# iangitonga/tinyllama.cpp

Hardware: AMD Instinct MI355X
Metric: decode tok/s TinyLlama-1.1B q4 ctx=2048, 1 GPU; achieved HBM GB/s vs peak (higher is better)
Workload: dtype q4 weights x q8 activations (int8 dot, f32 accumulate); 1 GPU; TinyLlama-1.1B q4 greedy single-token decode, batch 1 per GPU, steps end at n=2048 (BASELINE.json configs[3]); ctx=2048, graph=True, steps_per_graph_replay=4, kv_cache=q8 blocks (reference layout), argmax=device, parallelism=replicas x1

## Files before the change

### tinyllama.cpp_amd/csrc/gten_decode.hip

```cpp
#include "gten_dev.h"
#include "gten_rt.h"
#include "gten_hip_sample.h"

#include <cmath>
#include <vector>
#include <algorithm>

using namespace gtd;

extern __shared__ __attribute__((aligned(16))) uint8_t g_smem[];

#define DEC_CHUNK 256
#define DEC_MAX_LANES 4
#define DEC_ATT_MAXCH 8
#define GEMVM_F16_LDS_LIMIT 65536

static int g_only_family = -1;
#define DEC_LAUNCH(tag, kernel, grid, block, smem, ...)                                        \
    do {                                                                                       \
        if (g_only_family < 0 || g_only_family == (tag)) GTR_LAUNCH(tag, kernel, grid, block, smem, __VA_ARGS__); \
    } while (0)

#define DEC_LAUNCH_HOT(tag, kernel, grid, block, smem, hw, a) \
    DEC_LAUNCH(tag, kernel, grid, block, smem, (hw).w[0], (hw).w[1], (hw).w[2], (hw).w[3], (hw).w[4], (hw).w[5], (hw).w[6], a)

struct DecStep {
    int n;
    int advance;
    int stop;
};


struct ActStage {
    float* row;
    float* red;
    ActQ8 q8;
};

__device__ __forceinline__ ActStage carve_stage(int d)
{
    ActStage s;
    s.red = (float*)g_smem;
    s.row = (float*)(g_smem + 64);
    s.q8 = actq8_carve(g_smem + 64 + (size_t)d * 4, d >> 5);
    return s;
}
static size_t stage_bytes(int d) { return 64 + (size_t)d * 4 + (size_t)(d >> 5) * 40; }

enum { PRO_EMBED = 0, PRO_RESID = 1, PRO_ATT = 2, PRO_ATTW = 3, PRO_ACTQ8 = 4 };
enum { EPI_RAW = 0, EPI_SILUMUL = 1, EPI_STAGE = 2, EPI_STAGE_FRAG = 3 };

#define WXP_PLANES 8
#include "gten_decode_wx.h"
#include "gten_decode_wide_wx.h"
#include "gten_decode_ffn.h"
#include "gten_decode_wxp.h"
#include "gten_decode_attn.h"
#include "gten_decode_attn_exact64.h"
#include "gten_decode_attn_wide.h"
#include "gten_decode_attn_hm.h"
#include "gten_decode_sample.h"


using namespace gtr;

struct gten_hip_decoder {
    gten_hip_decoder_desc d;
    std::vector<gten_hip_layer_ptrs> layers;
    DecStep* step = nullptr;
    int32_t* tokens = nullptr;
    int32_t* result = nullptr;
    int32_t* ids_stage = nullptr;
    float *qkv_raw = nullptr, *proj_raw = nullptr, *down_raw = nullptr;
    float *scores = nullptr, *stats = nullptr, *att_part = nullptr;
    uint8_t *xbuf = nullptr, *hbuf = nullptr;
    float* act_f = nullptr;
    int8_t* act_q = nullptr;
    float* act_d = nullptr;
    int* act_sum = nullptr;
    float* best_val = nullptr;
    int* best_idx = nullptr;
    int n_best = 0;
    std::vector<DecStep> slots;
    int dev_n = -1;
    std::vector<int> dev_ns;
    int only_family = -1;
    int n_seq = 1;
    const void** kv_tab = nullptr;
    std::vector<const void*> kv_real;
    std::vector<char> kv_parked;
    void* dummy_kv = nullptr;
    int8_t* stg_q = nullptr;
    float* stg_d = nullptr;
    int* stg_sum = nullptr;
    float* stg_f = nullptr;
    float* logits_m = nullptr;
    float* gu_raw = nullptr;
    int n_chunks = 0;
    hipGraph_t graph = nullptr;
    hipGraphExec_t exec = nullptr;
    hipGraph_t graph_k = nullptr;
    hipGraphExec_t exec_k = nullptr;
    hipGraph_t graph_m[1 << DEC_MAX_LANES] = {}, graph_km[1 << DEC_MAX_LANES] = {};
    hipGraphExec_t exec_m[1 << DEC_MAX_LANES] = {}, exec_km[1 << DEC_MAX_LANES] = {};
    SampleParam* samp = nullptr;
    std::vector<SampleParam> samp_host;
    int n_sampling = 0;
    hipGraph_t s_graph = nullptr, s_graph_k = nullptr, s_graph_m[1 << DEC_MAX_LANES] = {}, s_graph_km[1 << DEC_MAX_LANES] = {};
    hipGraphExec_t s_exec = nullptr, s_exec_k = nullptr, s_exec_m[1 << DEC_MAX_LANES] = {}, s_exec_km[1 << DEC_MAX_LANES] = {};
    unsigned lane_mask = 0;
    int last_run_lanes = 0;
    const float2* rope = nullptr;
    float2* rope_now = nullptr;
    bool exact = false;
    bool persist_on = false;
    struct PersistState* persist = nullptr;
    uint8_t* hm = nullptr;
    size_t hm_seq_stride = 0, hm_cache_bytes = 0, hm_chunk_bytes = 0;
    std::vector<char> hm_dirty;
    unsigned long long hm_imports = 0, hm_import_launches = 0;
    unsigned long long watch_epoch = 0;
    bool watch_foreign = false;
    int lanes = 1;
    hipStream_t lane_stream[DEC_MAX_LANES] = {nullptr, nullptr, nullptr, nullptr};
    hipEvent_t lane_fork = nullptr, lane_join[DEC_MAX_LANES] = {nullptr, nullptr, nullptr, nullptr};
};

struct LaneBufs {
    int n_seq;
    DecStep* step; int32_t* tokens; int32_t* result; const SampleParam* samp;
    float *qkv_raw, *proj_raw, *down_raw, *scores, *stats, *att_part;
    uint8_t *xbuf, *hbuf;
    float* act_f; int8_t* act_q; float* act_d; int* act_sum;
    const void** kv_tab;
    int8_t* stg_q; float* stg_d; int* stg_sum; float* stg_f;
    float* logits_m; float* gu_raw; float2* rope_now;
};
static LaneBufs lane_bufs(const gten_hip_decoder* dc, int lane)
{
    const gten_hip_decoder_desc& d = dc->d;
    const size_t SL = (size_t)(dc->n_seq / dc->lanes), o = (size_t)lane * SL;
    const size_t E = (size_t)d.n_embd, F = (size_t)d.n_ffn, dh = E / d.n_heads, KV = dh * d.n_kv_heads, V = (size_t)d.n_vocab;
    const size_t planes = dc->n_seq >= 16 ? 2 : 1, H = (size_t)d.n_heads, C = (size_t)dc->n_chunks;
    LaneBufs b;
    b.n_seq = (int)SL;
    b.step = dc->step + o; b.tokens = dc->tokens + o * (d.max_ctx + 1); b.result = dc->result + o * (d.max_ctx + 2); b.samp = dc->samp + o;
    const size_t rplanes = dc->n_seq >= 16 ? (size_t)WXP_PLANES : 1;
    b.qkv_raw = dc->qkv_raw + o * rplanes * (E + 2 * KV);
    b.proj_raw = dc->proj_raw + o * rplanes * E; b.down_raw = dc->down_raw + o * rplanes * E;
    b.scores = dc->scores + o * H * d.max_ctx; b.stats = dc->stats + o * H * C * 2; b.att_part = dc->att_part + o * H * C * dh;
    b.xbuf = dc->xbuf + o * E * 4; b.hbuf = dc->hbuf + o * E * 4;
    b.act_f = dc->act_f + o * F; b.act_q = dc->act_q + o * 2 * F; b.act_d = dc->act_d + o * (F / 32); b.act_sum = dc->act_sum + o * (F / 32);
    b.kv_tab = dc->kv_tab ? dc->kv_tab + o * d.n_layers * 2 : nullptr;
    b.stg_q = dc->stg_q ? dc->stg_q + o * 2 * E : nullptr; b.stg_d = dc->stg_d ? dc->stg_d + o * (E / 32) : nullptr;
    b.stg_sum = dc->stg_sum ? dc->stg_sum + o * (E / 32) : nullptr; b.stg_f = dc->stg_f ? dc->stg_f + o * E : nullptr;
    b.logits_m = dc->logits_m ? dc->logits_m + o * V : nullptr; b.gu_raw = dc->gu_raw ? dc->gu_raw + o * planes * 2 * F : nullptr;
    b.rope_now = dc->rope_now + o * (dh / 2);
    return b;
}

static bool g_decode_exact = false;
static bool g_exact_now = false;
static bool g_lane_skip = false;
static bool g_kv_head_major = true;
extern "C" int gten_hip_set_kv_head_major(int on)
{
    g_kv_head_major = on != 0;
    return 0;
}
extern "C" int gten_hip_set_decode_exact(int on)
{
    g_decode_exact = on != 0;
    return 0;
}

static bool attention_grouped_ok(const AttnArgs& t, int n_seq)
{
    const int grp = t.n_heads / t.n_kv;
    const int min_seq = 8;
    if (t.adtype == GTEN_F16 && n_seq < 16) return false;
    return n_seq >= min_seq && (t.adtype == GTEN_Q8 || t.adtype == GTEN_F16) && t.d_head == 64 && (grp == 8 || grp == 4 || grp == 2 || grp == 1);
}

static int grp_shift1_of(int n_heads, int n_kv)
{
    const int grp = n_heads / n_kv;
    return (grp > 0 && (grp & (grp - 1)) == 0) ? __builtin_ctz(grp) + 1 : 0;
}

static bool attention_one_pass(int d_head);

static bool grouped_mm(const AttnArgs& t, int n_seq)
{
    return n_seq >= 16 && t.adtype == GTEN_Q8 && t.d_head == 64 && !g_exact_now;
}

static bool grouped_hm_f16(const AttnArgs& t, int n_seq)
{
    return n_seq >= 16 && t.adtype == GTEN_F16 && t.d_head == 64 && t.hm_k && !g_exact_now;
}

static bool grouped_one_pass(const AttnArgs& t, int n_seq)
{
    if (grouped_mm(t, n_seq) || grouped_hm_f16(t, n_seq)) return true;
    return attention_one_pass(t.d_head) && t.adtype == GTEN_Q8 && n_seq <= 8;
}

template <int GRP, int ADT>
static int launch_attention_g(const AttnArgs& t, int n_seq)
{
    constexpr size_t NW = (ADT == GTEN_Q8) ? 17 : 32;
    const dim3 grid(n_seq, t.n_chunks, t.n_kv);
    if constexpr (ADT == GTEN_Q8) if (grouped_mm(t, n_seq) && t.hm_k) {
        const int n_cq = (t.n_chunks + HM_WAVES - 1) / HM_WAVES;
        if (n_seq >= 128) DEC_LAUNCH(KT_DEC_ATTN_SCORE, (k_dec_attn_hm<GRP, true>), dim3(n_seq * n_cq * t.n_kv), dim3(64 * HM_WAVES), 2048, t, n_seq, n_cq);
        else DEC_LAUNCH(KT_DEC_ATTN_SCORE, (k_dec_attn_hm<GRP, false>), dim3(n_seq * n_cq * t.n_kv), dim3(64 * HM_WAVES), 2048, t, n_seq, n_cq);
        return 0;
    }
    if constexpr (ADT == GTEN_Q8) if (grouped_mm(t, n_seq)) {
        const size_t smem = (size_t)DEC_CHUNK * 68 + 2 * 8 * 264 * 2 + 16 * 64 + 32 * 4 + 8 * 4 + (size_t)4 * (DEC_MAXGRP + 2) * 2 + 128 + 128 * 4 + 80 + 64;
        GTR_REQUIRE((n_seq * t.n_chunks) % 8 == 0, "decoder: %d sequences x %d chunks is not a multiple of 8", n_seq, t.n_chunks);
        DEC_LAUNCH(KT_DEC_ATTN_SCORE, (k_dec_attn_mm_g<GRP>), dim3(n_seq * t.n_chunks * t.n_kv), dim3(256), smem, t, n_seq);
        return 0;
    }
    if constexpr (ADT == GTEN_Q8) if (grouped_one_pass(t, n_seq)) {
        constexpr size_t GP = (GRP + 1) / 2;
        const size_t smem = (size_t)(8 * GRP + 4 * GRP + 8 + 64) * 4 + (size_t)4 * (GRP + 2) * 2 + (size_t)(GRP + 2) * 64 + 16 +
// ... 19 lines not shown
        const size_t smem_m = (size_t)(128 + 16) * 4 + 128 + 128 + 64 + 16 + (size_t)17 * 64 * 2 + 64;
        DEC_LAUNCH(KT_DEC_ATTN_SCORE, (k_dec_attn_score_gm_f16<GRP>), grid, dim3(256), smem_m, t);
    } else if (ADT == GTEN_F16) {
        AttnArgs t1 = t;
        t1.grp_shift1 = grp_shift1_of(t.n_heads, t.n_kv);
        const AttnHotWords none{{0, 0, 0, 0, 0, 0, 0}};
        const size_t smem_s = (size_t)(16 + 3 * 64 + 16) * 4 + 32 + (size_t)3 * 64 + 64;
        DEC_LAUNCH_HOT(KT_DEC_ATTN_SCORE, (k_dec_attn_score64<GTEN_F16, true>), dim3(t.n_chunks, t.n_heads, n_seq), dim3(256), smem_s, none, t1);
    } else {
        DEC_LAUNCH(KT_DEC_ATTN_SCORE, (k_dec_attn_score_g<GRP, ADT>), grid, dim3(256), smem1, t);
    }
    if (exact) DEC_LAUNCH(KT_DEC_ATTN_PV, (k_dec_attn_pv_g<GRP, true, ADT>), grid, dim3(256), smem2, t);
    else DEC_LAUNCH(KT_DEC_ATTN_PV, (k_dec_attn_pv_g<GRP, false, ADT>), grid, dim3(256), smem2, t);
    return 0;
}

static int launch_attention_grouped(const AttnArgs& t, int n_seq)
{
    if (t.adtype == GTEN_Q8) {
        switch (t.n_heads / t.n_kv) {
        case 8: return launch_attention_g<8, GTEN_Q8>(t, n_seq);
        case 4: return launch_attention_g<4, GTEN_Q8>(t, n_seq);
        case 2: return launch_attention_g<2, GTEN_Q8>(t, n_seq);
        default: return launch_attention_g<1, GTEN_Q8>(t, n_seq);
        }
    }
    switch (t.n_heads / t.n_kv) {
    case 8: return launch_attention_g<8, GTEN_F16>(t, n_seq);
    case 4: return launch_attention_g<4, GTEN_F16>(t, n_seq);
    case 2: return launch_attention_g<2, GTEN_F16>(t, n_seq);
    default: return launch_attention_g<1, GTEN_F16>(t, n_seq);
    }
}

static bool attention_one_pass(int d_head)
{
    return d_head == 64 && !g_exact_now;
}

static int launch_attention(const AttnArgs& t0, dim3 agrid, size_t smem1)
{
    AttnArgs t = t0;
    t.grp_shift1 = grp_shift1_of(t.n_heads, t.n_kv);
    if (attention_one_pass(t.d_head)) {
        const size_t nw = (t.adtype == GTEN_Q8) ? 17 : 32;
        const size_t smem = 1152 + (size_t)2 * DEC_CHUNK * 4 + (size_t)DEC_CHUNK * nw * 4;
        const unsigned long long geo = (unsigned long long)(unsigned)t.kv_pitch | ((unsigned long long)(unsigned)t.max_ctx << 32);
        const unsigned long long heads = ((unsigned long long)(unsigned)t.n_heads << 32) | ((unsigned long long)(unsigned)t.n_kv << 40) |
                                         ((unsigned long long)(unsigned)t.grp_shift1 << 48);
        const AttnHotWords hw{{(unsigned long long)(uintptr_t)t.qkv_raw, (unsigned long long)(uintptr_t)t.rope_now, (unsigned long long)(uintptr_t)t.kcache,
                               (unsigned long long)(uintptr_t)t.step, geo, (unsigned long long)(unsigned)t.n_embd | heads, (unsigned long long)(uintptr_t)t.vcache}};
        const bool multi = agrid.z > 1 || t.kv_tab != nullptr;
        const dim3 g64(agrid.y, agrid.x, agrid.z);
        if (t.adtype == GTEN_Q8) {
            if (multi) DEC_LAUNCH_HOT(KT_DEC_ATTN_SCORE, (k_dec_attn_one64<GTEN_Q8, true>), g64, dim3(256), smem, hw, t);
            else DEC_LAUNCH_HOT(KT_DEC_ATTN_SCORE, (k_dec_attn_one64<GTEN_Q8, false>), g64, dim3(256), smem, hw, t);
        } else {
            if (multi) DEC_LAUNCH_HOT(KT_DEC_ATTN_SCORE, (k_dec_attn_one64<GTEN_F16, true>), g64, dim3(256), smem, hw, t);
            else DEC_LAUNCH_HOT(KT_DEC_ATTN_SCORE, (k_dec_attn_one64<GTEN_F16, false>), g64, dim3(256), smem, hw, t);
        }
        return 0;
    }
    if (t.d_head == 64) {
        const size_t nw = (t.adtype == GTEN_Q8) ? 17 : 32;
        const size_t smem2 = (size_t)2 * DEC_CHUNK * 4 + (size_t)DEC_CHUNK * nw * 4;
        const unsigned long long geo = (unsigned long long)(unsigned)t.kv_pitch | ((unsigned long long)(unsigned)t.max_ctx << 32);
        const unsigned long long heads = ((unsigned long long)(unsigned)t.n_heads << 32) | ((unsigned long long)(unsigned)t.n_kv << 40) |
                                         ((unsigned long long)(unsigned)t.grp_shift1 << 48);
        const AttnHotWords hs{{(unsigned long long)(uintptr_t)t.qkv_raw, (unsigned long long)(uintptr_t)t.rope_now, (unsigned long long)(uintptr_t)t.kcache,
                               (unsigned long long)(uintptr_t)t.step, geo, (unsigned long long)(unsigned)t.n_embd | heads, (unsigned long long)(uintptr_t)t.scores}};
        const AttnHotWords hp{{(unsigned long long)(uintptr_t)t.scores, (unsigned long long)(uintptr_t)t.stats, (unsigned long long)(uintptr_t)t.vcache,
                               (unsigned long long)(uintptr_t)t.step, geo, (unsigned long long)(unsigned)t.n_chunks | heads, (unsigned long long)(uintptr_t)t.att_part}};
        const bool multi = agrid.z > 1 || t.kv_tab != nullptr;
        const dim3 g64(agrid.y, agrid.x, agrid.z);
#define ATT_LAUNCH2(ADT, MULTI)                                                                                                          \
        do {                                                                                                                             \
            DEC_LAUNCH_HOT(KT_DEC_ATTN_SCORE, (k_dec_attn_score64<ADT, MULTI>), g64, dim3(256), smem1, hs, t);                           \
            DEC_LAUNCH_HOT(KT_DEC_ATTN_PV, (k_dec_attn_pv64<ADT, MULTI>), g64, dim3(256), smem2, hp, t);                                 \
        } while (0)
        if (t.adtype == GTEN_Q8) { if (multi) ATT_LAUNCH2(GTEN_Q8, true); else ATT_LAUNCH2(GTEN_Q8, false); }
        else { if (multi) ATT_LAUNCH2(GTEN_F16, true); else ATT_LAUNCH2(GTEN_F16, false); }
#undef ATT_LAUNCH2
        return 0;
    }
    DEC_LAUNCH(KT_DEC_ATTN_SCORE, k_dec_attn_score, agrid, dim3(256), smem1, t);
    DEC_LAUNCH(KT_DEC_ATTN_PV, k_dec_attn_pv, agrid, dim3(256), (size_t)2 * DEC_CHUNK * 4, t);
    return 0;
}

template <int WT, int PRO>
static GemvHotWords hot_of(const Gemv8Args& a)
{
    GemvHotWords hw;
    GemvHot& h = hw.h;
    if (PRO == PRO_RESID) { h.p0 = a.res_raw; h.p1 = a.res_a; h.p2 = a.norm_w; }
    else if (PRO == PRO_EMBED) { h.p0 = a.table; h.p1 = a.tokens; h.p2 = a.norm_w; }
    else if (PRO == PRO_ATT || PRO == PRO_ATTW) {
        h.p0 = a.att_part; h.p1 = (const void*)(uintptr_t)((unsigned)a.d_head_shift | ((unsigned)a.n_chunks << 8));
        h.p2 = (PRO == PRO_ATTW) ? a.att_stats : nullptr;
    }
    else { h.p0 = (WT == GTEN_F16) ? (const void*)a.act_f : (const void*)a.act_q; h.p1 = a.act_d; h.p2 = a.act_sum; }
    h.qs0 = a.qs[0]; h.ds0 = a.ds[0]; h.d_in = a.d_in; h.rows0 = a.rows[0]; h.step = a.step;
    return hw;
}

template <int WT, int PRO>
// ... 664 lines not shown
        }
        if (down_planes) {
            if ((rc = launch_wxp_f16(KT_DEC_GEMV_DOWN, (const uint16_t*)b.act_q, L.wdown, b.down_raw, F, E, S, E))) return rc;
        } else if ((rc = mmk(KT_DEC_GEMV_DOWN, b.act_q, b.act_d, b.down_raw, E, F, ks_of(F), L.wdown, E))) return rc;
    }
    Gemv8Args sf = base;
    sf.d_in = E; sf.res_a = hbuf; sf.res_raw = b.down_raw; sf.raw_stride = E; sf.norm_w = (const uint16_t*)d.final_norm;
    sf.raw_plane = (down_planes || ks_of(F) > 1) ? S * E : 0;
    sf.raw_nplanes = down_planes ? WXP_PLANES : 0;
    sf.act_q = b.stg_q; sf.act_d = b.stg_d; sf.act_sum = b.stg_sum; sf.act_f = b.stg_f;
    if ((rc = launch_stage_frag<WT, PRO_RESID>(KT_DEC_STAGE, sf, S))) return rc;
    if ((rc = mm(KT_DEC_GEMV_HEAD, b.stg_q, b.stg_d, b.stg_sum, b.logits_m, V, E, d.lm_head, V))) return rc;
    if (dc->n_sampling > 0)
        DEC_LAUNCH(KT_DEC_SAMPLE, k_dec_sample, dim3(S), dim3(SMP_THREADS), 0, (const float*)b.logits_m, V, V, b.samp,
                   b.step, b.result, d.max_ctx + 2, b.tokens, d.max_ctx + 1);
    else
        DEC_LAUNCH(KT_DEC_ARGMAX, k_dec_argmax, dim3(S), dim3(1024), 0, (const float*)b.logits_m, (const int*)nullptr,
                   V, b.step, b.result, V, d.max_ctx + 2, b.tokens, d.max_ctx + 1);
    return 0;
}

template <int WT>
static int enqueue_multi(gten_hip_decoder* dc, int lane)
{
    switch (dc->n_seq) {
    case 2: return enqueue_step_multi<WT, 2>(dc);
    case 4: return enqueue_step_multi<WT, 4>(dc);
    case 8: return enqueue_step_multi<WT, 8>(dc);
    }
    if (dc->n_seq >= 16) return enqueue_step_wide<WT>(dc, lane);
    return fail(-4, "decoder: n_seq %d not supported for this configuration", dc->n_seq);
}

#ifndef GTEN_WITH_PERSIST
#define GTEN_WITH_PERSIST 0
#endif
#if GTEN_WITH_PERSIST
#include "gten_decode_persist.h"
#else
struct PersistState {};
static bool g_persist_on = false;
extern "C" int gten_hip_set_decode_persistent(int on)
{
    if (on) return fail(-4, "set_decode_persistent: this library was built without the persistent step (-DGTEN_WITH_PERSIST=1, HISTORY.md)");
    return 0;
}
#endif

static int persist_prepare(gten_hip_decoder* dc);

static int enqueue_lane(gten_hip_decoder* dc, int lane)
{
    g_exact_now = dc->exact;
#if GTEN_WITH_PERSIST
    if (dc->persist_on && dc->n_seq == 1 && !dc->exact && (g_only_family < 0 || g_only_family == KT_DEC_PERSIST)) {
        if (int rc = persist_prepare(dc)) return rc;
        if (dc->persist) return persist_launch<GTEN_Q4>(dc->persist);
    }
#endif
    if (dc->n_seq > 1) {
        switch (dc->d.wdtype) {
        case GTEN_F16: return enqueue_multi<GTEN_F16>(dc, lane);
        case GTEN_Q8: return enqueue_multi<GTEN_Q8>(dc, lane);
        case GTEN_Q4: return enqueue_multi<GTEN_Q4>(dc, lane);
        }
    }
    switch (dc->d.wdtype) {
    case GTEN_F16: return enqueue_step_q8act<GTEN_F16>(dc);
    case GTEN_Q8: return enqueue_step_q8act<GTEN_Q8>(dc);
    case GTEN_Q4: return enqueue_step_q8act<GTEN_Q4>(dc);
    }
    return fail(-4, "decoder: bad weight dtype %d", dc->d.wdtype);
}

static int enqueue(gten_hip_decoder* dc, int count = 1)
{
    if (dc->lanes <= 1) {
        for (int i = 0; i < count; i++)
            if (int rc = enqueue_lane(dc, 0)) return rc;
        return 0;
    }
    const unsigned all = (1u << dc->lanes) - 1u, mask = (dc->lane_mask & all) ? (dc->lane_mask & all) : all;
    int g0 = 0;
    while (!((mask >> g0) & 1u)) g0++;
    const bool side = (mask & ~(1u << g0)) != 0;
    hipStream_t main_s = stream();
    if (side) {
        GTR_CHECK(hipEventRecord(dc->lane_fork, main_s));
        for (int g = g0 + 1; g < dc->lanes; g++)
            if ((mask >> g) & 1u) GTR_CHECK(hipStreamWaitEvent(dc->lane_stream[g], dc->lane_fork, 0));
    }
    int rc = 0;
    for (int g = g0; g < dc->lanes && !rc; g++) {
        if (!((mask >> g) & 1u)) continue;
        if (g != g0) gtr::stream_override(dc->lane_stream[g]);
        for (int i = 0; i < count && !rc; i++) rc = enqueue_lane(dc, g);
        gtr::stream_override(nullptr);
    }
    for (int g = g0 + 1; g < dc->lanes; g++) {
        if (!((mask >> g) & 1u)) continue;
        GTR_CHECK(hipEventRecord(dc->lane_join[g], dc->lane_stream[g]));
        GTR_CHECK(hipStreamWaitEvent(main_s, dc->lane_join[g], 0));
    }
    return rc;
}

static int decoder_build(gten_hip_decoder* dc, const gten_hip_decoder_desc& d, const gten_hip_layer_ptrs* layers,
                         const gten_hip_kv_ptrs* kv, int n_seq);

static int decoder_create_common(const gten_hip_decoder_desc* desc, const gten_hip_layer_ptrs* layers,
                                 const gten_hip_kv_ptrs* kv, int n_seq, gten_hip_decoder** out)
{
    GTR_NEED_INIT();
    GTR_REQUIRE(desc && layers && out, "decoder_create: null argument");
    const gten_hip_decoder_desc& d = *desc;
    GTR_REQUIRE(d.n_layers > 0 && d.n_heads > 0 && d.n_kv_heads > 0 && d.n_heads % d.n_kv_heads == 0, "decoder_create: bad head/layer counts");
    GTR_REQUIRE(d.n_embd % d.n_heads == 0, "decoder_create: n_embd %% n_heads != 0");
    const int dh = d.n_embd / d.n_heads;
    GTR_REQUIRE(dh == 32 || dh == 64, "decoder_create: fast path supports d_head 32 or 64 (got %d)", dh);
    GTR_REQUIRE(d.n_embd % 32 == 0 && d.n_ffn % 32 == 0 && d.n_embd <= 2048 && d.n_ffn <= 6144, "decoder_create: unsupported widths (n_embd <= 2048, n_ffn <= 6144)");
    GTR_REQUIRE(d.n_vocab > 0 && d.n_vocab <= 65535, "decoder_create: n_vocab %d outside [1, 65535] (row counts travel as 16-bit fields of the preloaded arguments)", d.n_vocab);
    GTR_REQUIRE(d.max_ctx > 0 && d.max_ctx <= GTEN_ROPE_MAX_POS, "decoder_create: max_ctx %d beyond the RoPE table", d.max_ctx);
    const bool pair_ok = (d.wdtype == GTEN_F16 && d.adtype == GTEN_F16) || ((d.wdtype == GTEN_Q8 || d.wdtype == GTEN_Q4) && d.adtype == GTEN_Q8);
    GTR_REQUIRE(pair_ok, "decoder_create: unsupported dtype pair (%d,%d) (tinyllama.cpp:258-265)", d.wdtype, d.adtype);
    GTR_REQUIRE(d.embed && d.final_norm && d.lm_head, "decoder_create: null model pointer");
    const bool wide = n_seq >= 16;
    GTR_REQUIRE(n_seq == 1 || n_seq == 2 || n_seq == 4 || n_seq == 8 || (wide && n_seq <= 64 && n_seq % 16 == 0) ||
                (n_seq > 64 && n_seq <= 64 * DEC_MAX_LANES && n_seq % 64 == 0) || (n_seq > 256 && n_seq <= 128 * DEC_MAX_LANES && n_seq % 128 == 0),
                "decoder_create: n_seq %d not in {1, 2, 4, 8, 16, 32, 48, 64, 128, 192, 256, 384, 512}", n_seq);
    GTR_REQUIRE(!wide || (d.n_ffn % 256 == 0 && d.n_embd % 256 == 0 && (dh * d.n_kv_heads) % 16 == 0),
                "decoder_create: n_seq >= 16 runs the W.x on the matrix cores: n_embd and n_ffn %% 256 == 0");
    GTR_REQUIRE(!wide || d.wdtype != GTEN_Q8 || d.n_ffn <= MMV_MAXP * 512,
                "decoder_create: q8 weights with n_seq >= 16 want n_ffn <= %d (the down projection's weight slab), got %d", MMV_MAXP * 512, d.n_ffn);
    GTR_REQUIRE(n_seq == 1 || (kv && dh == 64), "decoder_create: multi-sequence decode needs the cache table and d_head 64");
    GTR_REQUIRE(n_seq > 1 || d.logits, "decoder_create: null logits pointer");
    if (n_seq > 1)
        for (size_t i = 0; i < (size_t)n_seq * d.n_layers; i++)
            GTR_REQUIRE(kv[i].kcache && kv[i].vcache, "decoder_create: null cache pointer (sequence %zu, layer %zu)", i / d.n_layers, i % d.n_layers);
    auto* dc = new gten_hip_decoder;
    if (const int rc = decoder_build(dc, d, layers, kv, n_seq)) {
        char msg[512];
        snprintf(msg, sizeof(msg), "%s", gten_hip_last_error());
        gten_hip_decoder_destroy(dc);
        return fail(rc, "%s", msg);
    }
    *out = dc;
    return 0;
}

static int decoder_build(gten_hip_decoder* dc, const gten_hip_decoder_desc& d, const gten_hip_layer_ptrs* layers,
                         const gten_hip_kv_ptrs* kv, int n_seq)
{
    const int dh = d.n_embd / d.n_heads;
    const bool wide = n_seq >= 16;
    dc->d = d;
    dc->n_seq = n_seq;
    dc->exact = g_decode_exact;
    dc->persist_on = g_persist_on;
    {
        const bool can128 = !g_decode_exact && n_seq % 128 == 0 &&
                            ((d.wdtype != GTEN_F16 && d.adtype == GTEN_Q8) || (d.wdtype == GTEN_F16 && d.adtype == GTEN_F16 && d.n_embd == 2048));
        const int lane_rows = can128 ? 128 : 64;
        const int lanes = (n_seq + lane_rows - 1) / lane_rows;
        GTR_REQUIRE(lanes <= DEC_MAX_LANES, "decoder_create: %d sequences need %d lanes of %d (at most %d: f16 weights and the exact forms run lanes of 64)",
                    n_seq, lanes, lane_rows, DEC_MAX_LANES);
        dc->lanes = lanes;
    }
    for (int g = 1; g < dc->lanes; g++) {
        GTR_CHECK(hipStreamCreateWithFlags(&dc->lane_stream[g], hipStreamNonBlocking));
        GTR_CHECK(hipEventCreateWithFlags(&dc->lane_join[g], hipEventDisableTiming));
    }
    if (dc->lanes > 1) GTR_CHECK(hipEventCreateWithFlags(&dc->lane_fork, hipEventDisableTiming));
    dc->layers.assign(layers, layers + d.n_layers);
    dc->n_chunks = (d.max_ctx + DEC_CHUNK - 1) / DEC_CHUNK;
    static_assert(GTEN_ROPE_MAX_POS <= DEC_ATT_MAXCH * DEC_CHUNK, "max_ctx (checked above) bounds the attention chunks the consumers request up front");
    const int E = d.n_embd, F = d.n_ffn, KV = dh * d.n_kv_heads;
    const size_t S = (size_t)n_seq;
    GTR_CHECK(hipMalloc((void**)&dc->step, S * sizeof(DecStep)));
    GTR_CHECK(hipMemset(dc->step, 0, S * sizeof(DecStep)));
    GTR_CHECK(hipMalloc((void**)&dc->tokens, S * (size_t)(d.max_ctx + 1) * 4));
    GTR_CHECK(hipMemset(dc->tokens, 0, S * (size_t)(d.max_ctx + 1) * 4));
    GTR_CHECK(hipMalloc((void**)&dc->result, S * (size_t)(d.max_ctx + 2) * 4));
    GTR_CHECK(hipMemset(dc->result, 0, S * (size_t)(d.max_ctx + 2) * 4));
    GTR_CHECK(hipMalloc((void**)&dc->samp, S * sizeof(SampleParam)));
    GTR_CHECK(hipMemset(dc->samp, 0, S * sizeof(SampleParam)));
    dc->samp_host.assign(S, SampleParam{});
    const size_t planes = wide ? 2 : 1;
    GTR_CHECK(hipMalloc((void**)&dc->qkv_raw, (wide ? (size_t)WXP_PLANES : 1) * S * (size_t)(E + 2 * KV) * 4));
    GTR_CHECK(hipMalloc((void**)&dc->proj_raw, (wide ? (size_t)WXP_PLANES : 1) * S * (size_t)E * 4));
    GTR_CHECK(hipMalloc((void**)&dc->down_raw, (wide ? (size_t)WXP_PLANES : 1) * S * (size_t)E * 4));
    GTR_CHECK(hipMalloc((void**)&dc->scores, S * (size_t)d.n_heads * d.max_ctx * 4));
    GTR_CHECK(hipMalloc((void**)&dc->stats, (S * (size_t)d.n_heads * dc->n_chunks * 2 + 16) * 4));
    GTR_CHECK(hipMemset(dc->stats, 0, (S * (size_t)d.n_heads * dc->n_chunks * 2 + 16) * 4));
    GTR_CHECK(hipMalloc((void**)&dc->att_part, S * (size_t)d.n_heads * dc->n_chunks * dh * 4));
    GTR_CHECK(hipMalloc((void**)&dc->xbuf, S * (size_t)E * 4));
    GTR_CHECK(hipMalloc((void**)&dc->hbuf, S * (size_t)E * 4));
    const size_t stage_rows = wide ? 2 * ((S + 15) / 16 * 16) : S;
    GTR_CHECK(hipMalloc((void**)&dc->act_q, stage_rows * (size_t)F));
    GTR_CHECK(hipMemset(dc->act_q, 0, stage_rows * (size_t)F));
    GTR_CHECK(hipMalloc((void**)&dc->act_d, S * (size_t)(F / 32) * 4));
    GTR_CHECK(hipMalloc((void**)&dc->act_sum, S * (size_t)(F / 32) * 4));
    GTR_CHECK(hipMalloc((void**)&dc->act_f, S * (size_t)F * 4));
    {
        const int r = (n_seq == 1) ? (d.wdtype == GTEN_F16 ? 4 : 8) : (d.wdtype == GTEN_F16 ? 2 : 4);
        dc->n_best = ((d.n_vocab + 8 * r - 1) / (8 * r)) * 8;
    }
    GTR_CHECK(hipMalloc((void**)&dc->best_val, S * (size_t)dc->n_best * 4));
    GTR_CHECK(hipMalloc((void**)&dc->best_idx, S * (size_t)dc->n_best * 4));
    if (n_seq > 1) {
        GTR_CHECK(hipMalloc((void**)&dc->stg_q, stage_rows * (size_t)E));
// ... 852 lines not shown
```

### tinyllama.cpp_amd/csrc/gten_decode_attn.h

```cpp

struct AttnArgs {
    const DecStep* step;
    const float* qkv_raw;
    uint8_t* kcache; uint8_t* vcache; size_t kv_pitch;
    float* scores;
    float* stats;
    float* att_part;
    const float2* rope;
    const float2* rope_now;
    int adtype, n_heads, n_kv, d_head, max_ctx, n_chunks, n_embd;
    int grp_shift1;
    const void* const* kv_tab; int layer, n_layers;
    int qkv_stride, scores_stride, stats_stride, part_stride;
    int qkv_plane;
    int qkv_nplanes;
    uint8_t* hm_k; size_t hm_seq_stride, hm_cache_bytes;
};

typedef const unsigned __attribute__((address_space(1)))* gmem_u32;
__device__ __forceinline__ gmem_u32 as_global(const void* p) { return (gmem_u32)(uintptr_t)p; }

__device__ __forceinline__ AttnArgs attn_for_seq(const AttnArgs& a, int seq)
{
    AttnArgs t = a;
// ... 349 lines not shown
    p[threadIdx.x] = pr;
    __syncthreads();

    const int e = threadIdx.x & 63, cg = threadIdx.x >> 6;
    const uint8_t* vb = (const uint8_t*)vl;
    float o = 0.f;
    if (ADT == GTEN_Q8) {
        const int qoff = (e < 32) ? 2 + e : 36 + (e - 32), doff = (e < 32) ? 0 : 34;
        if (len == DEC_CHUNK) {
            float pp[2][8];
            int qv[2][8];
            unsigned dv[2][8];
            auto fetch = [&](int r, int slot) {
#pragma unroll
                for (int u = 0; u < 8; u++) {
                    const uint8_t* row = vb + (size_t)(cg + 4 * (8 * r + u)) * 68;
                    pp[slot][u] = p[cg + 4 * (8 * r + u)];
                    qv[slot][u] = (int)(int8_t)row[qoff];
                    dv[slot][u] = *(const uint16_t*)(row + doff);
                }
            };
            fetch(0, 0);
#pragma unroll
            for (int r = 0; r < DEC_CHUNK / 32; r++) {
                if (r + 1 < DEC_CHUNK / 32) fetch(r + 1, (r + 1) & 1);
                __builtin_amdgcn_sched_barrier(0);
#pragma unroll
                for (int u = 0; u < 8; u++) o += pp[r & 1][u] * ((float)qv[r & 1][u] * h2f((uint16_t)dv[r & 1][u]));
                __builtin_amdgcn_sched_barrier(0);
            }
        } else {
#pragma unroll 8
            for (int cl = cg; cl < len; cl += 4) {
                const uint8_t* row = vb + (size_t)cl * 68;
                o += p[cl] * ((float)(int8_t)row[qoff] * h2f(*(const uint16_t*)(row + doff)));
            }
        }
    } else {
        for (int cl = cg; cl < len; cl += 4) o += p[cl] * h2f(((const uint16_t*)(vb + (size_t)cl * 128))[e]);
    }
    part[threadIdx.x] = o;
    __syncthreads();
    if (threadIdx.x < dh) {
        float r = 0.f;
        for (int gi = 0; gi < 4; gi++) r += part[gi * dh + threadIdx.x];
        a.att_part[((size_t)h * a.n_chunks + chunk) * dh + threadIdx.x] = r;
    }
    if (threadIdx.x == 64) {
        a.stats[((size_t)h * a.n_chunks + chunk) * 2 + 0] = mx;
        a.stats[((size_t)h * a.n_chunks + chunk) * 2 + 1] = sm;
    }
}


__device__ __forceinline__ void dec_pick_commit(DecStep* step, int32_t* __restrict__ result, int32_t* __restrict__ tokens, int idx)
{
    const int n = step->n;
    result[n] = idx;
    const int adv = step->advance;
    if (adv & 2) tokens[n] = idx;
    const int stop = step->stop;
    if ((adv & 1) && (stop <= 0 || n < stop)) step->n = n + 1;
}

__global__ __launch_bounds__(1024) void k_dec_argmax(const float* __restrict__ vals0, const int* __restrict__ idxs0, int count,
                                                     DecStep* step0, int32_t* __restrict__ result0, int cand_stride, int result_stride,
                                                     int32_t* __restrict__ tokens0, int tok_stride)
{
    const float* vals = vals0 + (size_t)blockIdx.x * cand_stride;
    const int* idxs = idxs0 ? idxs0 + (size_t)blockIdx.x * cand_stride : nullptr;
    DecStep* step = step0 + blockIdx.x;
    int32_t* result = result0 + (size_t)blockIdx.x * result_stride;
    __shared__ float bv[16];
    __shared__ int bi[16];
    float best = -INFINITY;
    int idx = 0x7fffffff;
    for (int i = threadIdx.x; i < count; i += blockDim.x) {
        const float v = vals[i];
        const int vi = idxs ? idxs[i] : i;
        if (v > best || (v == best && vi < idx)) { best = v; idx = vi; }
    }
#pragma unroll
    for (int o = 32; o > 0; o >>= 1) {
        const float ov = __shfl_xor(best, o, 64);
        const int oi = __shfl_xor(idx, o, 64);
        if (ov > best || (ov == best && oi < idx)) { best = ov; idx = oi; }
    }
    const int lane = threadIdx.x & 63, wid = threadIdx.x >> 6;
    if (lane == 0) { bv[wid] = best; bi[wid] = idx; }
    __syncthreads();
    if (threadIdx.x == 0) {
        for (int w = 1; w < (int)(blockDim.x >> 6); w++)
            if (bv[w] > best || (bv[w] == best && bi[w] < idx)) { best = bv[w]; idx = bi[w]; }
        if (idx == 0x7fffffff) idx = 0;
        dec_pick_commit(step, result, tokens0 + (size_t)blockIdx.x * tok_stride, idx);
    }
}
```

### tinyllama.cpp_amd/hipabi.py

```python
import ctypes as C
import os

import numpy as np

from . import build as _build

I32, F16, F32, Q8, Q4 = 0, 1, 2, 3, 4


class GtenHipError(RuntimeError):
    pass


def _sig(lib, name, res, args):
    f = getattr(lib, name)
    f.restype = res
    f.argtypes = args
    return f


class DeviceBuffer:

    def __init__(self, api, nbytes):
        self.api = api
# ... 9 lines not shown
        buf.upload(arr)
        return buf

    def upload(self, arr, offset=0):
        arr = np.ascontiguousarray(arr)
        assert offset + arr.nbytes <= self.nbytes
        self.api._check(self.api._h2d(self.ptr + offset, arr.ctypes.data_as(C.c_void_p), arr.nbytes))

    def download(self, dtype=np.uint8, shape=None, offset=0, nbytes=None):
        nbytes = self.nbytes - offset if nbytes is None else nbytes
        out = np.empty(nbytes, dtype=np.uint8)
        self.api._check(self.api._d2h(out.ctypes.data_as(C.c_void_p), self.ptr + offset, nbytes))
        out = out.view(dtype)
        return out.reshape(shape) if shape is not None else out

    def zero(self, byte=0):
        self.api._check(self.api._memset(self.ptr, byte, self.nbytes))

    def free(self):
        if self.ptr:
            self.api._check(self.api._free(self.ptr))
            self.ptr = None

    def __del__(self):
        try:
            self.free()
        except Exception:
            pass


class BlockDesc(C.Structure):
    _fields_ = ([(k, C.c_int) for k in ("adtype", "wdtype", "n_embd", "n_heads", "n_kv_heads", "n_ffn")] +
                [(k, C.c_void_p) for k in ("attn_norm_w", "wq", "wk", "wv", "wo", "ffn_norm_w", "wgate", "wup", "wdown", "inp",
                                           "attn_norm_out", "q", "k", "v", "attn_out", "o", "h", "ffn_norm_out", "gate", "up", "down", "out")])


class GtenHip:

    SYMBOLS = [
        "gten_hip_device_count", "gten_hip_init", "gten_hip_last_error", "gten_hip_stream", "gten_hip_sync", "gten_hip_select_stream", "gten_hip_stream_wait", "gten_hip_stream_idle",
        "gten_hip_malloc", "gten_hip_free", "gten_hip_memset", "gten_hip_memcpy_h2d", "gten_hip_memcpy_d2h",
        "gten_hip_memcpy_d2d", "gten_hip_prof_enable", "gten_hip_prof_read", "gten_hip_prof_family_name",
        "gten_hip_selftest_q8scale", "gten_hip_row_bytes", "gten_hip_pack_weight", "gten_hip_token_embed",
        "gten_hip_block_rows", "gten_hip_set_block_rows", "gten_hip_matmul_2d", "gten_hip_rms_norm", "gten_hip_rotary_emb", "gten_hip_silu", "gten_hip_mul",
        "gten_hip_add", "gten_hip_qkv_attn", "gten_hip_argmax_row", "gten_hip_set_prefill_exact", "gten_hip_set_decode_exact", "gten_hip_set_decode_persistent", "gten_hip_persist_status", "gten_hip_set_row_segments", "gten_hip_row_segments_ok", "gten_hip_copy_ranges",
        "gten_hip_decoder_create", "gten_hip_decoder_destroy", "gten_hip_decoder_set_tokens",
        "gten_hip_decoder_step", "gten_hip_decoder_steps", "gten_hip_decoder_generate", "gten_hip_decoder_generate_multi", "gten_hip_decoder_step_ragged", "gten_hip_decoder_result", "gten_hip_decoder_time_family",
        "gten_hip_decoder_create_multi", "gten_hip_decoder_set_tokens_seq", "gten_hip_decoder_result_seq",
        "gten_hip_decoder_logits_seq",
        "gten_hip_decoder_lane_info", "gten_hip_set_lane_skip", "gten_hip_decoder_slot_start", "gten_hip_decoder_slot_start_until", "gten_hip_decoder_slot_park", "gten_hip_decoder_slot_bind", "gten_hip_decoder_slots_apply", "gten_hip_decoder_run", "gten_hip_decoder_run_lanes", "gten_hip_decoder_slot_ids", "gten_hip_decoder_slot_ids_all",
        "gten_hip_set_kv_head_major", "gten_hip_decoder_kv_info", "gten_hip_kv_watch_selftest", "gten_hip_set_ffn_streamed", "gten_hip_set_wx_planes",
    ]
    SAMPLE_SYMBOLS = ["gten_hip_decoder_set_sampling", "gten_hip_sample_rows"]

    def __init__(self, path=None):
        path = path or _build.HIP_LIB
        if not os.path.exists(path):
            raise GtenHipError(f"{path} is missing: run __graft_entry__.build() (hipcc --offload-arch=gfx950)")
        self.path = path
        self.lib = L = C.CDLL(path, mode=C.RTLD_GLOBAL)
        vp, sz, ci = C.c_void_p, C.c_size_t, C.c_int
        self._count = _sig(L, "gten_hip_device_count", ci, [])
        self._init = _sig(L, "gten_hip_init", ci, [ci])
        self._err = _sig(L, "gten_hip_last_error", C.c_char_p, [])
        self._stream = _sig(L, "gten_hip_stream", vp, [])
        self._sync = _sig(L, "gten_hip_sync", ci, [])
        self._selftest_q8 = _sig(L, "gten_hip_selftest_q8scale", ci, [C.POINTER(C.c_ulonglong), C.POINTER(C.c_ulonglong)])
        self._malloc = _sig(L, "gten_hip_malloc", ci, [C.POINTER(vp), sz])
        self._free = _sig(L, "gten_hip_free", ci, [vp])
        self._memset = _sig(L, "gten_hip_memset", ci, [vp, ci, sz])
        self._h2d = _sig(L, "gten_hip_memcpy_h2d", ci, [vp, vp, sz])
        self._d2h = _sig(L, "gten_hip_memcpy_d2h", ci, [vp, vp, sz])
        self._d2d = _sig(L, "gten_hip_memcpy_d2d", ci, [vp, vp, sz])
        self._row_bytes = _sig(L, "gten_hip_row_bytes", sz, [ci, ci])
        self._prof_enable = _sig(L, "gten_hip_prof_enable", ci, [ci])
        self._prof_read = _sig(L, "gten_hip_prof_read", ci, [ci, C.POINTER(ci), C.POINTER(C.c_double)])
        self._prof_name = _sig(L, "gten_hip_prof_family_name", C.c_char_p, [ci])
        self._pack = _sig(L, "gten_hip_pack_weight", ci, [vp, ci, ci, ci, vp])
        self._embed = _sig(L, "gten_hip_token_embed", ci, [vp, ci, ci, vp, vp, ci, sz, ci, ci, ci])
        self._matmul = _sig(L, "gten_hip_matmul_2d", ci, [vp, ci, sz, vp, ci, vp, ci, sz, ci, ci, ci, ci])
        self._rms = _sig(L, "gten_hip_rms_norm", ci, [vp, ci, sz, vp, vp, sz, ci, ci, ci])
        self._rope = _sig(L, "gten_hip_rotary_emb", ci, [vp, ci, sz, ci, ci, ci, ci])
        self._silu = _sig(L, "gten_hip_silu", ci, [vp, vp, ci, sz, ci, ci, ci])
        self._mul = _sig(L, "gten_hip_mul", ci, [vp, vp, vp, ci, sz, ci, ci, ci])
        self._add = _sig(L, "gten_hip_add", ci, [vp, vp, vp, ci, sz, ci, ci, ci])
        self._attn = _sig(L, "gten_hip_qkv_attn", ci, [vp, vp, vp, vp, ci, sz, sz, sz, ci, ci, ci, ci, ci])
        self._prefill_exact = _sig(L, "gten_hip_set_prefill_exact", ci, [ci])
        self._block_rows = _sig(L, "gten_hip_block_rows", ci, [C.POINTER(BlockDesc), ci, ci])
        self._set_block_rows = _sig(L, "gten_hip_set_block_rows", ci, [ci])
        self._decode_exact = _sig(L, "gten_hip_set_decode_exact", ci, [ci])
        self._decode_persistent = _sig(L, "gten_hip_set_decode_persistent", ci, [ci])
        self._kv_head_major = _sig(L, "gten_hip_set_kv_head_major", ci, [ci])
        self._kv_watch_selftest = _sig(L, "gten_hip_kv_watch_selftest", ci, [])
        self._ffn_streamed = _sig(L, "gten_hip_set_ffn_streamed", ci, [ci])
        self._wx_planes = _sig(L, "gten_hip_set_wx_planes", ci, [ci])
        self._lane_skip = _sig(L, "gten_hip_set_lane_skip", ci, [ci])
        self._persist_status = _sig(L, "gten_hip_persist_status", ci, [C.POINTER(ci), C.POINTER(C.c_ulonglong), C.POINTER(C.c_uint), C.c_void_p, ci])
        self._set_row_segments = _sig(L, "gten_hip_set_row_segments", ci, [C.c_void_p, ci])
        self._copy_ranges = _sig(L, "gten_hip_copy_ranges", ci, [C.c_void_p, ci])
        self._set_sampling = _sig(L, "gten_hip_decoder_set_sampling", ci, [vp, ci, ci, C.c_float, C.c_uint64, C.c_uint32])
        self._sample_rows = _sig(L, "gten_hip_sample_rows", ci, [vp, ci, ci, C.c_longlong, vp, vp, C.c_uint64, vp, vp, vp])
        self.initialised = False

    def _check(self, rc):
        if rc != 0:
            raise GtenHipError(f"gten_hip error {rc}: {self._err().decode(errors='replace')}")

    def device_count(self):
        return self._count()

    def init(self, device=0):
        if self.device_count() <= device:
            raise GtenHipError(f"no MI355X visible (device_count={self.device_count()}, asked for {device}); "
                               "there is no CPU fallback for the gten_hip path")
        self._check(self._init(device))
        self.initialised = True
        return self

    def sync(self):
        self._check(self._sync())

    def selftest_q8scale(self):
        a, b = C.c_ulonglong(0), C.c_ulonglong(0)
        self._check(self._selftest_q8(C.byref(a), C.byref(b)))
        return a.value, b.value

    def stream(self):
        return self._stream()

    def set_row_segments(self, starts):
        if not starts:
            self._check(self._set_row_segments(None, 0))
            return
        a = np.ascontiguousarray(starts, dtype=np.int32)
        self._check(self._set_row_segments(a.ctypes.data_as(C.c_void_p), len(a) - 1))

    def copy_ranges(self, ranges):
        class R(C.Structure):
            _fields_ = [("dst", C.c_void_p), ("src", C.c_void_p), ("bytes", C.c_size_t)]
        arr = (R * len(ranges))(*[R(int(d), int(s), int(b)) for d, s, b in ranges])
        self._check(self._copy_ranges(C.cast(arr, C.c_void_p), len(ranges)))

    def sample_rows(self, logits, n_rows, n_vocab, row_stride, top_k, temp, seed, stream, position):
        def per_row(v, dt):
            a = np.ascontiguousarray(np.broadcast_to(np.asarray(v, dtype=dt), (n_rows,)))
            return a, a.ctypes.data_as(C.c_void_p)
        (k, kp), (t, tp), (s, sp), (p, pp) = (per_row(top_k, np.int32), per_row(temp, np.float32), per_row(stream, np.uint32),
                                              per_row(position, np.int32))
        out = DeviceBuffer(self, max(4 * n_rows, 4))
        self._check(self._sample_rows(logits.ptr, n_rows, n_vocab, row_stride, kp, tp, C.c_uint64(int(seed)), sp, pp, out.ptr))
        return out.download(np.int32)[:n_rows].copy()

    def sample_rows_rc(self, logits, n_rows, n_vocab, row_stride, top_k, temp, seed=0, stream=0, position=1):
        k, t = np.full(max(n_rows, 1), top_k, np.int32), np.full(max(n_rows, 1), temp, np.float32)
        s, p = np.full(max(n_rows, 1), stream, np.uint32), np.full(max(n_rows, 1), position, np.int32)
        out = DeviceBuffer(self, 4 * max(n_rows, 1))
        return self._sample_rows(logits.ptr, n_rows, n_vocab, row_stride, k.ctypes.data_as(C.c_void_p), t.ctypes.data_as(C.c_void_p),
                                 C.c_uint64(int(seed)), s.ctypes.data_as(C.c_void_p), p.ctypes.data_as(C.c_void_p), out.ptr)

    def set_decode_exact(self, on):
        self._check(self._decode_exact(1 if on else 0))

    def set_kv_head_major(self, on):
        self._check(self._kv_head_major(1 if on else 0))

    def set_ffn_streamed(self, on):
        self._check(self._ffn_streamed(1 if on else 0))

    def set_wx_planes(self, on):
        self._check(self._wx_planes(1 if on else 0))

    def kv_watch_selftest(self):
        return int(self._kv_watch_selftest())

    def set_decode_persistent(self, on):
        self._check(self._decode_persistent(1 if on else 0))

    def set_lane_skip(self, on):
        self._check(self._lane_skip(1 if on else 0))

    def persist_status(self, n_stamps=0):
        nd, nl, ab = C.c_int(0), C.c_ulonglong(0), C.c_uint(0)
        st = (C.c_uint * max(n_stamps, 1))()
        self._check(self._persist_status(C.byref(nd), C.byref(nl), C.byref(ab), C.cast(st, C.c_void_p) if n_stamps else None, n_stamps))
        return nd.value, nl.value, ab.value, list(st)[:n_stamps]

    def set_prefill_exact(self, on):
        self._check(self._prefill_exact(1 if on else 0))

    def select_stream(self, idx):
        self._check(self.lib.gten_hip_select_stream(int(idx)))

    def set_block_rows(self, on):
        self._check(self._set_block_rows(1 if on else 0))

    def block_rows(self, n, start_pos, ints, bufs):
        d = BlockDesc()
        for k, v in ints.items():
            setattr(d, k, int(v))
        for k, v in bufs.items():
            setattr(d, k, v.ptr)
        rc = self._block_rows(C.byref(d), n, start_pos)
        if rc == 1:
            return False
        self._check(rc)
        return True

    def prof_enable(self, on):
        self._check(self._prof_enable(1 if on else 0))

    def prof_family_index(self, wanted):
        fam = 0
        while True:
            name = self._prof_name(fam)
# ... 80 lines not shown
```

Baseline: 2059 tok/s.

## Add one-pass attention variant that preloads V rows and transposes into LDS

Adds a new single-chunk decode attention kernel that loads both K and V rows for each context position up front in registers. It dequantises V into a padded LDS tile and computes the P·V product column-wise with strided-padded reads, instead of the previous layout. It becomes the default for the non-multi path, and the old kernel stays reachable through a new 'classic' toggle. The aim is to overlap V fetch latency with the score/softmax phase and to cut LDS bank conflicts, at the cost of much larger dynamic shared memory (about 70KB) and so lower occupancy. It also calls hipFuncSetAttribute on every launch.

```diff
diff --git a/include/gten_hip_ab.h b/include/gten_hip_ab.h
--- /dev/null
+++ b/include/gten_hip_ab.h
@@ -0,0 +1,11 @@
+#pragma once
+
+#ifdef __cplusplus
+extern "C" {
+#endif
+
+int gten_hip_set_decode_attn_classic(int on);
+
+#ifdef __cplusplus
+}
+#endif
diff --git a/tinyllama.cpp_amd/csrc/gten_decode.hip b/tinyllama.cpp_amd/csrc/gten_decode.hip
--- a/tinyllama.cpp_amd/csrc/gten_decode.hip
+++ b/tinyllama.cpp_amd/csrc/gten_decode.hip
@@ -1,6 +1,7 @@
 #include "gten_dev.h"
 #include "gten_rt.h"
 #include "gten_hip_sample.h"
+#include "gten_hip_ab.h"
 
 #include <cmath>
 #include <vector>
@@ -11,6 +12,8 @@
 extern __shared__ __attribute__((aligned(16))) uint8_t g_smem[];
 
 #define DEC_CHUNK 256
+#define ATT1V_VROW 68
+#define ATT1V_PCOL 72
 #define DEC_MAX_LANES 4
 #define DEC_ATT_MAXCH 8
 #define GEMVM_F16_LDS_LIMIT 65536
@@ -113,6 +116,7 @@
     const float2* rope = nullptr;
     float2* rope_now = nullptr;
     bool exact = false;
+    bool attn_classic = false;
     bool persist_on = false;
     struct PersistState* persist = nullptr;
     uint8_t* hm = nullptr;
@@ -173,6 +177,13 @@
     g_decode_exact = on != 0;
     return 0;
 }
+static bool g_attn_classic = false;
+static bool g_attn_classic_now = false;
+extern "C" int gten_hip_set_decode_attn_classic(int on)
+{
+    g_attn_classic = on != 0;
+    return 0;
+}
 
 static bool attention_grouped_ok(const AttnArgs& t, int n_seq)
 {
@@ -298,6 +309,17 @@
                                (unsigned long long)(uintptr_t)t.step, geo, (unsigned long long)(unsigned)t.n_embd | heads, (unsigned long long)(uintptr_t)t.vcache}};
         const bool multi = agrid.z > 1 || t.kv_tab != nullptr;
         const dim3 g64(agrid.y, agrid.x, agrid.z);
+        if (!multi && !g_attn_classic_now) {
+            const size_t smem_v = 1152 + (size_t)(4 * ATT1V_PCOL + DEC_CHUNK) * 4 + (size_t)DEC_CHUNK * ATT1V_VROW * 4;
+            if (t.adtype == GTEN_Q8) {
+                GTR_CHECK(hipFuncSetAttribute((const void*)k_dec_attn_one64v<GTEN_Q8>, hipFuncAttributeMaxDynamicSharedMemorySize, (int)smem_v));
+                DEC_LAUNCH_HOT(KT_DEC_ATTN_SCORE, k_dec_attn_one64v<GTEN_Q8>, g64, dim3(256), smem_v, hw, t);
+            } else {
+                GTR_CHECK(hipFuncSetAttribute((const void*)k_dec_attn_one64v<GTEN_F16>, hipFuncAttributeMaxDynamicSharedMemorySize, (int)smem_v));
+                DEC_LAUNCH_HOT(KT_DEC_ATTN_SCORE, k_dec_attn_one64v<GTEN_F16>, g64, dim3(256), smem_v, hw, t);
+            }
+            return 0;
+        }
         if (t.adtype == GTEN_Q8) {
             if (multi) DEC_LAUNCH_HOT(KT_DEC_ATTN_SCORE, (k_dec_attn_one64<GTEN_Q8, true>), g64, dim3(256), smem, hw, t);
             else DEC_LAUNCH_HOT(KT_DEC_ATTN_SCORE, (k_dec_attn_one64<GTEN_Q8, false>), g64, dim3(256), smem, hw, t);
@@ -1068,6 +1090,7 @@
 static int enqueue_lane(gten_hip_decoder* dc, int lane)
 {
     g_exact_now = dc->exact;
+    g_attn_classic_now = dc->attn_classic;
 #if GTEN_WITH_PERSIST
     if (dc->persist_on && dc->n_seq == 1 && !dc->exact && (g_only_family < 0 || g_only_family == KT_DEC_PERSIST)) {
         if (int rc = persist_prepare(dc)) return rc;
@@ -1172,6 +1195,7 @@
     dc->d = d;
     dc->n_seq = n_seq;
     dc->exact = g_decode_exact;
+    dc->attn_classic = g_attn_classic;
     dc->persist_on = g_persist_on;
     {
         const bool can128 = !g_decode_exact && n_seq % 128 == 0 &&
diff --git a/tinyllama.cpp_amd/csrc/gten_decode_attn.h b/tinyllama.cpp_amd/csrc/gten_decode_attn.h
--- a/tinyllama.cpp_amd/csrc/gten_decode_attn.h
+++ b/tinyllama.cpp_amd/csrc/gten_decode_attn.h
@@ -425,6 +425,190 @@
     }
 }
 
+template <int ADT>
+__global__ __launch_bounds__(256) void k_dec_attn_one64v(const unsigned long long h0, const unsigned long long h1, const unsigned long long h2,
+                                                        const unsigned long long h3, const unsigned long long h4, const unsigned long long h5,
+                                                        const unsigned long long h6, const AttnArgs a0)
+{
+    AttnArgs a = a0;
+    a.qkv_raw = from_word<float>(h0); a.rope_now = from_word<float2>(h1); a.kcache = (uint8_t*)from_word<uint8_t>(h2);
+    a.step = from_word<DecStep>(h3); a.kv_pitch = (size_t)(unsigned)(h4 & 0xffffffffull); a.max_ctx = (int)(h4 >> 32);
+    a.n_embd = (int)(unsigned)(h5 & 0xffffffffull); a.n_heads = (int)((h5 >> 32) & 0xffu); a.n_kv = (int)((h5 >> 40) & 0xffu); a.grp_shift1 = (int)(h5 >> 48);
+    a.vcache = (uint8_t*)from_word<uint8_t>(h6);
+    constexpr int dh = 64, nblk = 2;
+    constexpr int NW = (ADT == GTEN_Q8) ? 17 : 32;
+    constexpr int VS = ATT1V_VROW, PS = ATT1V_PCOL;
+    const int h = blockIdx.y, chunk = blockIdx.x, c0 = chunk * DEC_CHUNK;
+    const int grp = a.grp_shift1 ? (1 << (a.grp_shift1 - 1)) : a.n_heads / a.n_kv, g = a.grp_shift1 ? (h >> (a.grp_shift1 - 1)) : h / grp;
+    const int kv_dim = a.n_kv * dh;
+    const size_t head_bytes = (ADT == GTEN_Q8) ? (size_t)nblk * GTEN_Q8_BYTES : (size_t)dh * 2;
+
+    float* red = (float*)g_smem;
+    float* qf = red + 16 + dh;
+    float* kf = qf + dh;
+    float* qd = kf + dh;
+    float* kd = qd + 8;
+    uint16_t* d16 = (uint16_t*)(kd + 8);
+    int8_t* qi8 = (int8_t*)(d16 + 16);
+    int8_t* ki8 = qi8 + dh;
+    int8_t* vi8 = ki8 + dh;
+    float* pt = (float*)(g_smem + 1152);
+    float* part = pt + 4 * PS;
+    float* vf = part + DEC_CHUNK;
+
+    const int c = c0 + threadIdx.x;
+    const int t = threadIdx.x & 63, pw = threadIdx.x >> 6;
+    const int roff = (pw == 1) ? a.n_embd + g * dh : (pw == 2) ? a.n_embd + kv_dim + g * dh : h * dh;
+    const float raw = a.qkv_raw[roff + t];
+    const float2 rot = a.rope_now[t & 31];
+    __builtin_amdgcn_sched_barrier(0);
+    const int cs = min(c, a.max_ctx - 1);
+    const unsigned pitch_w = (unsigned)(a.kv_pitch >> 2);
+    const gmem_u32 kp = as_global(a.kcache + (size_t)g * head_bytes) + (unsigned)cs * pitch_w;
+    unsigned kw[NW];
+    unsigned vw[NW];
+    {
+        const gmem_u32 vp = as_global(a.vcache + (size_t)g * head_bytes) + (unsigned)cs * pitch_w;
+        typedef unsigned u4u __attribute__((ext_vector_type(4), aligned(4)));
+#pragma unroll
+        for (int j = 0; j + 4 <= NW; j += 4) {
+            const u4u kq = *(const __attribute__((address_space(1))) u4u*)(kp + j);
+            const u4u vq = *(const __attribute__((address_space(1))) u4u*)(vp + j);
+            kw[j] = kq.x; kw[j + 1] = kq.y; kw[j + 2] = kq.z; kw[j + 3] = kq.w;
+            vw[j] = vq.x; vw[j + 1] = vq.y; vw[j + 2] = vq.z; vw[j + 3] = vq.w;
+        }
+#pragma unroll
+        for (int j = NW & ~3; j < NW; j++) { kw[j] = kp[j]; vw[j] = vp[j]; }
+    }
+    __builtin_amdgcn_sched_barrier(0);
+    const int n = a.step->n, pos = n - 1;
+    if (c0 >= n) return;
+
+    const bool has_new = (pos >= c0) && (pos < c0 + DEC_CHUNK);
+    const bool writer = has_new && (h == g * grp);
+    float vnew = 0.f;
+    if (pw < 3) {
+        int8_t* dq = (pw == 0) ? qi8 : (pw == 1) ? ki8 : vi8;
+        float* dd = (pw == 0) ? qd : (pw == 1) ? kd : kd + 4;
+        const float v = head_prep_cs(raw, true, pw != 2, rot, dh, ADT, dq, dd, d16 + 4 * pw);
+        if (pw == 0) qf[t] = v;
+        if (pw == 1) kf[t] = v;
+        if (pw == 2) vnew = v;
+        if (pw >= 1 && writer) {
+            uint8_t* row = ((pw == 1) ? a.kcache : a.vcache) + (size_t)pos * a.kv_pitch + (size_t)g * head_bytes;
+            if (ADT == GTEN_Q8) {
+                uint8_t* blk = row + (size_t)(t >> 5) * GTEN_Q8_BYTES;
+                store_global<uint8_t>(blk + 2 + (t & 31), (uint8_t)dq[t]);
+                if ((t & 31) == 0) store_global<uint16_t>(blk, d16[4 * pw + (t >> 5)]);
+            } else {
+                store_global<uint16_t>((uint16_t*)row + t, f2h(v));
+            }
+        }
+    }
+    __syncthreads();
+
+    const float scale = 1.0f / sqrtf((float)dh);
+    float acc = 0.f;
+    if (ADT == GTEN_Q8) {
+        const int* qi = (const int*)qi8;
+        int isum = 0;
+#pragma unroll
+        for (int j = 0; j < 8; j++) isum = dot4(qi[j], (int)__builtin_amdgcn_alignbit(kw[j + 1], kw[j], 16), isum);
+        acc += (float)isum * (qd[0] * h2f((uint16_t)(kw[0] & 0xffffu)));
+        isum = 0;
+#pragma unroll
+        for (int j = 0; j < 8; j++) isum = dot4(qi[8 + j], (int)kw[9 + j], isum);
+        acc += (float)isum * (qd[1] * h2f((uint16_t)(kw[8] >> 16)));
+    } else {
+#pragma unroll
+        for (int j = 0; j < 32; j++) {
+            acc += qf[2 * j] * h2f((uint16_t)(kw[j] & 0xffffu));
+            acc += qf[2 * j + 1] * h2f((uint16_t)(kw[j] >> 16));
+        }
+    }
+    if (has_new) {
+        float accn = 0.f;
+        if (ADT == GTEN_Q8) {
+            const int* qi = (const int*)qi8;
+            const int* ki = (const int*)ki8;
+#pragma unroll
+            for (int b = 0; b < nblk; b++) {
+                int isum = 0;
+#pragma unroll
+                for (int j = 0; j < 8; j++) isum = dot4(qi[b * 8 + j], ki[b * 8 + j], isum);
+                accn += (float)isum * (qd[b] * kd[b]);
+            }
+        } else {
+            for (int e = 0; e < dh; e++) accn += qf[e] * kf[e];
+        }
+        if (c == pos) acc = accn;
+    }
+    const float sc = (c < n) ? acc * scale : -INFINITY;
+
+    if (c != pos) {
+        const bool live = c < n;
+        float4* dst = (float4*)(vf + threadIdx.x * VS);
+#pragma unroll
+        for (int j = 0; j < 16; j++) {
+            float f[4];
+#pragma unroll
+            for (int i = 0; i < 4; i++) {
+                const int e = 4 * j + i;
+                float x;
+                if (ADT == GTEN_Q8) {
+                    const int b = (e < 32) ? 2 + e : 4 + e;
+                    const int q = (int)(int8_t)(uint8_t)(vw[b >> 2] >> (8 * (b & 3)));
+                    const float d = h2f((uint16_t)((e < 32) ? (vw[0] & 0xffffu) : (vw[8] >> 16)));
+                    x = (float)q * d;
+                } else {
+                    x = h2f((uint16_t)((e & 1) ? (vw[e >> 1] >> 16) : (vw[e >> 1] & 0xffffu)));
+                }
+                f[i] = live ? x : 0.f;
+            }
+            dst[j] = make_float4(f[0], f[1], f[2], f[3]);
+        }
+    }
+    if (has_new && pw == 2) vf[(pos - c0) * VS + t] = vnew;
+
+    const float mx = block_max_n<4>(sc, red);
+    const float ex = (c < n) ? expf(sc - mx) : 0.f;
+    const float sm = block_sum_n<4>(ex, red + 4);
+
+    float pr = (c < n) ? ex / sm : 0.f;
+    if (ADT == GTEN_Q8) {
+        const Q8Scale s8 = q8_scale_from_absmax(max32(fabsf(pr)));
+        if (c < n) pr = (float)q8_round(pr, s8.scale) * s8.ddeq;
+    } else {
+        pr = h2f(f2h(pr));
+    }
+    pt[(threadIdx.x & 3) * PS + (threadIdx.x >> 2)] = pr;
+    __syncthreads();
+
+    const int e = threadIdx.x & 63, cg = threadIdx.x >> 6;
+    const float* vcol = vf + cg * VS + e;
+    const float4* pc = (const float4*)(pt + cg * PS);
+    float o = 0.f;
+#pragma unroll
+    for (int j = 0; j < DEC_CHUNK / 16; j++) {
+        const float4 p4 = pc[j];
+        o = o + p4.x * vcol[(4 * j + 0) * 4 * VS];
+        o = o + p4.y * vcol[(4 * j + 1) * 4 * VS];
+        o = o + p4.z * vcol[(4 * j + 2) * 4 * VS];
+        o = o + p4.w * vcol[(4 * j + 3) * 4 * VS];
+    }
+    part[threadIdx.x] = o;
+    __syncthreads();
+    if (threadIdx.x < dh) {
+        float r = 0.f;
+        for (int gi = 0; gi < 4; gi++) r += part[gi * dh + threadIdx.x];
+        a.att_part[((size_t)h * a.n_chunks + chunk) * dh + threadIdx.x] = r;
+    }
+    if (threadIdx.x == 64) {
+        a.stats[((size_t)h * a.n_chunks + chunk) * 2 + 0] = mx;
+        a.stats[((size_t)h * a.n_chunks + chunk) * 2 + 1] = sm;
+    }
+}
+
 
 __device__ __forceinline__ void dec_pick_commit(DecStep* step, int32_t* __restrict__ result, int32_t* __restrict__ tokens, int idx)
 {
diff --git a/tinyllama.cpp_amd/hipabi.py b/tinyllama.cpp_amd/hipabi.py
--- a/tinyllama.cpp_amd/hipabi.py
+++ b/tinyllama.cpp_amd/hipabi.py
@@ -85,6 +85,7 @@
         "gten_hip_set_kv_head_major", "gten_hip_decoder_kv_info", "gten_hip_kv_watch_selftest", "gten_hip_set_ffn_streamed", "gten_hip_set_wx_planes",
     ]
     SAMPLE_SYMBOLS = ["gten_hip_decoder_set_sampling", "gten_hip_sample_rows"]
+    AB_SYMBOLS = ["gten_hip_set_decode_attn_classic"]
 
     def __init__(self, path=None):
         path = path or _build.HIP_LIB
@@ -122,6 +123,7 @@
         self._block_rows = _sig(L, "gten_hip_block_rows", ci, [C.POINTER(BlockDesc), ci, ci])
         self._set_block_rows = _sig(L, "gten_hip_set_block_rows", ci, [ci])
         self._decode_exact = _sig(L, "gten_hip_set_decode_exact", ci, [ci])
+        self._decode_attn_classic = _sig(L, "gten_hip_set_decode_attn_classic", ci, [ci])
         self._decode_persistent = _sig(L, "gten_hip_set_decode_persistent", ci, [ci])
         self._kv_head_major = _sig(L, "gten_hip_set_kv_head_major", ci, [ci])
         self._kv_watch_selftest = _sig(L, "gten_hip_kv_watch_selftest", ci, [])
@@ -193,6 +195,9 @@
 
     def set_decode_exact(self, on):
         self._check(self._decode_exact(1 if on else 0))
+
+    def set_decode_attn_classic(self, on):
+        self._check(self._decode_attn_classic(1 if on else 0))
 
     def set_kv_head_major(self, on):
         self._check(self._kv_head_major(1 if on else 0))
```

New measurement: 2103 tok/s, median of 6. 2.1% higher.
